# Contingencyy/CPUGPUPathtracing

Hardware: AMD Instinct MI355X
Metric: Mrays/sec @ 1920x1080, 256 spp (dragon glTF stand-in) (higher is better)
Workload: dtype f32

## Files before the change

cpugpupathtracing_amd/_native.py:

```python
from __future__ import annotations

import ctypes as C
import os

from ._paths import LIB_PATH

ABI_VERSION = 2
CGPT_OK, CGPT_ERR_INVALID, CGPT_ERR_HIP, CGPT_ERR_NO_SCENE, CGPT_ERR_UNSUPPORTED, CGPT_ERR_NO_DEVICE = range(6)
OBJECT_MESH, OBJECT_SPHERE, OBJECT_PLANE, OBJECT_TRIANGLE = 0, 1, 2, 3
MODE_COMPARISON, MODE_BRUTE_FORCE, MODE_ADVANCED = 0, 1, 2
DEBUG_NONE, DEBUG_RAY_DEPTH, DEBUG_BVH_DEPTH = 0, 1, 2
KERNEL_AUTO, KERNEL_MEGAKERNEL, KERNEL_WAVEFRONT, KERNEL_PERSISTENT = 0, 1, 2, 3
RENDER_COUNTERS = 1
CTX_FORCE_COLLECTIVE, CTX_GATHER_PEER_COPY = 1, 2
BUILD_NAIVE, BUILD_SAH_INTERVALS, BUILD_SAH_PRIMITIVES = 0, 1, 2
BUILD_SAH_BINNED = 3
DENOISE_DEMODULATE_ALBEDO = 1
TRACE_COUNTERS, TRACE_REVERSED = 1, 2
TEMPORAL_KEEP_VIEW_DEPENDENT = 1
TEMPORAL_FOLLOW_TRANSFORMS = 4
VARIANCE_TEMPORAL = 1
SKIN_MAX_JOINTS = 1024

f3 = C.c_float * 3
# ... 202 lines not shown
    "cgpth_scene_get_smooth_normals": (C.c_int, [_vp, _up, C.c_uint32]),
    "cgpth_scene_set_transform": (C.c_int, [_vp, C.c_uint32, C.POINTER(C.c_float)]),
    "cgpth_scene_get_transforms": (C.c_int, [_vp, C.POINTER(C.c_float), C.c_uint32]),
    "cgpth_scene_set_camera": (C.c_int, [_vp, _fp, _fp, C.c_float, C.c_float]),
    "cgpth_scene_set_settings": (C.c_int, [_vp, C.POINTER(Settings)]),
    "cgpth_scene_rebuild_bvh": (C.c_int, [_vp, C.c_uint32, C.c_int]),
    "cgpth_scene_refit_mesh": (C.c_int, [_vp, C.c_uint32, C.POINTER(Triangle), C.c_uint32]),
    "cgpth_skin_triangles": (C.c_int, [C.POINTER(Triangle), _u16p, _fp, C.c_uint32, _fp, C.c_uint32, C.POINTER(Triangle)]),
    "cgpth_scene_skin_mesh": (C.c_int, [_vp, C.c_uint32, C.POINTER(Triangle), _u16p, _fp, C.c_uint32, _fp, C.c_uint32]),
    "cgpth_scene_update_primitive": (C.c_int, [_vp, C.c_uint32, C.POINTER(Object)]),
    "cgpth_scene_bvh_info": (C.c_int, [_vp, C.c_uint32, C.POINTER(BvhInfo)]),
    "cgpth_scene_bvh_export": (C.c_int, [_vp, C.c_uint32, C.POINTER(BvhNode), _up]),
    "cgpth_scene_flatten": (C.c_int, [_vp, C.POINTER(SceneDesc)]),
    "cgpth_scene_get_camera": (C.c_int, [_vp, C.POINTER(Camera)]),
    "cgpth_scene_get_settings": (C.c_int, [_vp, C.POINTER(Settings)]),
    "cgpth_write_ppm": (C.c_int, [C.c_char_p, _up, C.c_uint32, C.c_uint32]),
    "cgpth_write_pfm": (C.c_int, [C.c_char_p, _fp, C.c_uint32, C.c_uint32, C.c_uint32]),
    "cgpth_write_accumulator": (C.c_int, [C.c_char_p, _fp, C.c_uint32, C.c_uint32, C.c_uint32]),
    "cgpth_read_accumulator": (C.c_int, [C.c_char_p, _fp, _up, C.c_uint32, C.c_uint32]),
    "cgpth_fast_div": (C.c_uint32, [C.c_uint32, C.c_uint32]),
    "cgpth_motion_records": (C.c_uint32, [_fp, C.c_uint32, _fp, C.c_uint32, _fp]),
    "cgpth_shade_item_blocks": (C.c_uint32, [C.c_uint32, C.c_uint32, C.c_uint32]),
    "cgpth_shade_segment_blocks": (C.c_uint32, [C.c_uint32, C.c_uint32, C.c_uint32]),
    "cgpth_scene_layout": (C.c_int, [C.POINTER(SceneDesc), C.POINTER(SceneLayoutView)]),
    "cgpth_scene_layout_instanced": (C.c_int, [C.POINTER(SceneDesc), C.POINTER(SceneLayoutView)]),
    "cgpth_scene_layout_transformed": (C.c_int, [C.POINTER(SceneDesc), C.POINTER(C.c_float), C.c_uint32, C.POINTER(SceneLayoutView)]),
    "cgpth_scene_permute_objects": (C.c_int, [_vp, _up, C.c_uint32]),
    "cgpth_top_level": (C.c_int, [C.POINTER(SceneDesc), C.POINTER(TopLevelView)]),
    "cgpth_top_level_transforms": (C.c_int, [C.POINTER(C.c_float), C.c_uint32, C.POINTER(TopLevelView)]),
    "cgpth_top_level_refit": (C.c_int, [C.c_uint32, C.POINTER(Triangle), C.c_uint32, C.POINTER(TopLevelView)]),
    "cgpth_top_level_primitive": (C.c_int, [C.c_uint32, C.POINTER(Object), C.POINTER(TopLevelView)]),
}

DEBUG_PROTOTYPES = {
    "cgpt_debug_live_device_bytes": (C.c_uint64, []),
}

_lib = None


class NativeLibraryError(RuntimeError):
    pass


def lib() -> C.CDLL:
    global _lib
# ... 19 lines not shown
```

cpugpupathtracing_amd/csrc/device/persistent_kernel.hip:

```cpp
#include <hip/hip_runtime.h>

#include <algorithm>
#include <cstdint>
#include <cstdlib>
#include <new>

#include "cpugpupt_abi.h"
#include "device_scene.h"
#include "fast_div.h"
#include "rt_device.hpp"
#include "shade_device.hpp"
#include "trace_steps.hpp"
#include "accumulate.hpp"
#include "launch_common.h"

namespace cgpt {

using namespace dev;

hipStream_t CtxStream(cgpt_ctx* ctx);
void** CtxPersistentSlot(cgpt_ctx* ctx);
hipEvent_t CtxStartEvent(cgpt_ctx* ctx);
void PersistentFree(void* state);

// ... 359 lines not shown
    LAUNCH_TRY(hipEventRecord(CtxStartEvent(ctx), stream));
    LAUNCH_TRY(hipMemsetAsync(h->work_counters.p, 0, work_words * sizeof(uint32_t), stream));
    const TraceTune tt = { h->tune.refill_idle, h->tune.inner_repeat, h->tune.leaf_repeat, 1u, h->tune.obj_shift, top_records, 0u, h->tune.lds_tris, h->tune.tail_lanes, 0u };

    if (n_streams == 2) {
        LAUNCH_TRY(hipEventRecord(h->begin, stream));
        for (int i = 0; i < 2; ++i) LAUNCH_TRY(hipStreamWaitEvent(h->streams[i], h->begin, 0));
    }
    int launches = 0;
    uint32_t k = 0;
    for (uint32_t done = 0; done < args_in.n_samples; done += batch, ++k) {
        const uint32_t s = n_streams == 2 ? k & 1u : 0u;
        hipStream_t st = n_streams == 2 ? h->streams[s] : stream;
        const uint32_t bn = std::min(batch, args_in.n_samples - done);
        const uint32_t bfirst = args_in.first_sample + done;
        PtDev pt{};
        pt.st_en = h->st_en[s].p;
        pt.brute = brute ? h->brute.p + (size_t)s * (h->brute.n / n_streams) : nullptr;
        pt.stack_overflow = h->overflow.p + (size_t)s * (h->overflow.n / n_streams);
        pt.n_paths = n_pixels * bn;
        pt.g.n_pixels = n_pixels; pt.g.tiles_x = tiles_x; pt.g.div_tiles_x = MakeFastDiv(tiles_x); pt.g.div_n_pixels = MakeFastDiv(n_pixels);
        pt.shade_shift = h->tune.shade_shift;
        pt.g.order = h->tune.path_order; pt.g.n_samples = bn; pt.g.div_samples = MakeFastDiv(bn);
        pt.work = h->work_counters.p + (size_t)k * kWorkCounters * 8u;
        work_sizes(pt.n_paths, grid.x * (kTraceBlock / 64u), h->tune.fine_rounds, h->tune.chunk, pt.coarse, pt.fine_below);
        LAUNCH_TRY(hipEventRecord(NextEvent(h->ev), st));
        hipLaunchKernelGGL(kPtKernels[v.ris][level][v.count][brute][tail], grid, trace_block, lds, st, args_in, pt, bfirst, tt);
        LAUNCH_TRY(hipEventRecord(NextEvent(h->ev), st));
        if (n_streams == 2 && k > 0) LAUNCH_TRY(hipStreamWaitEvent(st, h->acc_done[(k - 1u) & 1u], 0));
        hipLaunchKernelGGL(pt_accumulate, dim3(std::min((n_pixels + 255u) / 256u, h->n_cus * 8u)), block, 0, st, args_in, (const float4*)pt.st_en, pt.g, bfirst, bn);
        if (n_streams == 2) LAUNCH_TRY(hipEventRecord(h->acc_done[s], st));
        LAUNCH_TRY(hipGetLastError());
        launches += 2;
    }
    if (n_streams == 2 && k > 0) LAUNCH_TRY(hipStreamWaitEvent(stream, h->acc_done[(k - 1u) & 1u], 0));
    return launches;
}

}
```

cpugpupathtracing_amd/csrc/device/trace_steps.hpp:

```cpp
#pragma once
#include <hip/hip_runtime.h>

#include "device_scene.h"
#include "fast_div.h"
#include "rt_device.hpp"

namespace cgpt {
namespace dev {

static constexpr uint32_t kStartObject = 0x40000000u;
static constexpr uint32_t kIdle = 0x40000001u;
#ifndef CGPT_LDS_STACK_LEVELS
#define CGPT_LDS_STACK_LEVELS 16
#endif
static constexpr uint32_t kLdsStackLevels = CGPT_LDS_STACK_LEVELS;
#ifndef CGPT_TRACE_BLOCK
#define CGPT_TRACE_BLOCK 256
#endif
static constexpr uint32_t kTraceBlock = CGPT_TRACE_BLOCK;
static constexpr uint32_t kRing = 128;
static constexpr uint32_t kLdsObjects = 31;
static constexpr uint32_t kKindEnd = 0xFFFFFFFFu;
static constexpr uint32_t kTopStride = 20;
static constexpr uint32_t kLdsTopMax = 127;
// ... 60 lines not shown

typedef float nt_f4 __attribute__((ext_vector_type(4)));
__device__ __forceinline__ float4 ld_stream(const float4* p)
{
    const nt_f4 v = __builtin_nontemporal_load(reinterpret_cast<const nt_f4*>(p));
    float4 r; r.x = v.x; r.y = v.y; r.z = v.z; r.w = v.w; return r;
}
__device__ __forceinline__ void st_stream(float4* p, float4 v)
{
    nt_f4 x; x.x = v.x; x.y = v.y; x.z = v.z; x.w = v.w;
    __builtin_nontemporal_store(x, reinterpret_cast<nt_f4*>(p));
}
__device__ __forceinline__ uint32_t ld_stream(const uint32_t* p) { return __builtin_nontemporal_load(p); }
__device__ __forceinline__ void st_stream(uint32_t* p, uint32_t v) { __builtin_nontemporal_store(v, p); }

enum PathOrder : uint32_t { kSampleMajor = 0, kTileMajor = 1, kPixelMajor = 2 };
struct PathGrid {
    uint32_t n_pixels;
    uint32_t tiles_x;
    FastDiv div_tiles_x, div_n_pixels;
    uint32_t n_samples;
    FastDiv div_samples;
    uint32_t order;
};
__device__ __forceinline__ void path_split(const PathGrid& g, uint32_t pid, uint32_t& sample, uint32_t& pixel)
{
    if (g.order == kPixelMajor) {
        pixel = fast_div(pid, g.div_samples);
        sample = pid - pixel * g.n_samples;
    } else if (g.order == kTileMajor) {
        const uint32_t b = pid >> 6, tile = fast_div(b, g.div_samples);
        sample = b - tile * g.n_samples;
        pixel = (tile << 6) | (pid & 63u);
    } else {
        sample = fast_div(pid, g.div_n_pixels);
        pixel = pid - sample * g.n_pixels;
    }
}
__device__ __forceinline__ uint32_t path_id(const PathGrid& g, uint32_t sample, uint32_t pixel)
{
    if (g.order == kPixelMajor) return pixel * g.n_samples + sample;
    return g.order == kTileMajor ? ((((pixel >> 6) * g.n_samples + sample) << 6) | (pixel & 63u)) : sample * g.n_pixels + pixel;
}
__device__ __forceinline__ bool pixel_of_index(const DevRenderArgs& a, const PathGrid& g, uint32_t p, uint32_t& px, uint32_t& py, uint32_t& local_row)
{
    const uint32_t tile = p >> 6, l = p & 63u;
    const uint32_t ty = fast_div(tile, g.div_tiles_x);
    const uint32_t tx = tile - ty * g.tiles_x;
    px = tx * 8u + (l & 7u);
    local_row = ty * 8u + (l >> 3);
    py = GlobalRow(local_row, a.band_first, a.band_h, a.band_stride);
    return px < a.width && local_row < a.n_rows;
}
__device__ __forceinline__ bool primary_ray(const DevRenderArgs& args, const PathGrid& g, uint32_t pid, uint32_t batch_first, Ray& ray, uint32_t& rng, uint32_t& px_out,
                                            uint32_t& pixel_out)
{
    uint32_t s, p;
    path_split(g, pid, s, p);
    pixel_out = p;
    uint32_t px, py, local_row;
    if (!pixel_of_index(args, g, p, px, py, local_row)) return false;
    px_out = px;
    rng = pcg_seed(py * args.width + px, batch_first + s, args.seed);
    ray = camera_ray(args.camera, (float)px * (1.0f / (float)args.width), (float)py * (1.0f / (float)args.height));
    return true;
}
__device__ __forceinline__ bool primary_ray(const DevRenderArgs& args, const PathGrid& g, uint32_t pid, uint32_t batch_first, Ray& ray, uint32_t& rng, uint32_t& px_out)
{
    uint32_t pixel_unused;
    return primary_ray(args, g, pid, batch_first, ray, rng, px_out, pixel_unused);
}
__device__ __forceinline__ bool pixel_ray(const DevRenderArgs& args, const PathGrid& g, uint32_t p, Ray& ray)
{
// ... 330 lines not shown
```

cpugpupathtracing_amd/csrc/device/wavefront_kernels.hip:

```cpp
#include <hip/hip_runtime.h>

#include <algorithm>
#include <cstdint>
#include <cstddef>
#include <cstdlib>
#include <cstring>
#include <new>
#include <type_traits>
#include <vector>

#include "cpugpupt_abi.h"
#include "ctx_internal.h"
#include "device_scene.h"
#include "fast_div.h"
#include "rt_device.hpp"
#include "shade_device.hpp"
#include "shade_items.h"
#include "trace_steps.hpp"
#include "accumulate.hpp"
#include "launch_common.h"

namespace cgpt {

using namespace dev;

hipStream_t CtxStream(cgpt_ctx* ctx);
void** CtxWavefrontSlot(cgpt_ctx* ctx);
hipEvent_t CtxStartEvent(cgpt_ctx* ctx);

extern __shared__ uint32_t lds_dyn[];

static constexpr uint32_t kMaxBands = 128;

struct WfDev {
    float4* A; float4* B; float4* C;
    float4* st_tp; float4* st_en;
    float4* px_hit;
    float4* brute;
    uint8_t* hit_flag;
    uint32_t* list_ext; uint32_t* list_sh;
// ... 557 lines not shown
                off += n; base += total;
            }
            if (seg == 0u) wf.plan[sh ? 1 : 0] = base;
        }
        __syncthreads();
        const uint32_t* src = (sh ? wf.seg_sh : wf.seg_ext) + (size_t)seg * wf.seg_cap;
        uint32_t* const list = sh ? wf.list_sh : wf.list_ext;
        for (uint32_t b = wave_in_block; b < wf.n_bands; b += 4u) {
            const uint32_t n = s_n[b], n4 = n & ~3u;
            uint32_t* dst = list + s_dst[b];
            const uint32_t* run = src + s_src[b];
            for (uint32_t i = lane * 4u; i < n4; i += 256u) *reinterpret_cast<u4a4*>(dst + i) = *reinterpret_cast<const u4a4*>(run + i);
            if (lane < n - n4) dst[n4 + lane] = run[n4 + lane];
        }
    }
}

__global__ void __launch_bounds__(256) wf_accumulate(const DevRenderArgs args, const WfDev wf, uint32_t batch_first, uint32_t batch_n)
{
    accumulate_batch<true>(args, wf.st_en, wf.g, batch_first, batch_n, wf.px_hit);
}

static constexpr uint32_t kMaxPools = 8;

struct WfTuning {
    uint32_t pools = 8;
    uint32_t batch = 0;
    uint32_t max_batch = 512;
    uint32_t pool_paths_mi = 512;
    uint32_t budget_gib = 96;
    uint32_t refill_idle = 16;
    uint32_t leaf_repeat = 4;
    uint32_t inner_repeat = 20;
    uint32_t obj_repeat = 1;
    uint32_t obj_shift = 0;
    uint32_t top_records = kLdsTopMax;
    uint32_t max_trace_blocks = 64;
    uint32_t max_shade_blocks = 5;
    uint32_t shade_chunk = 4;
    uint32_t shade_chunk_banded = 32;
    uint32_t shadow_any_hit = 1;
    uint32_t lds_tris = 1;
    uint32_t first_lean = 1;
    uint32_t trace_events = 1;
    uint32_t path_order = 2;
    uint32_t retire_misses = 1;
    uint32_t bands_min_paths = 32u << 20;
    uint32_t bands = 32;
    uint32_t spec_dedupe = 1;
// ... 49 lines not shown
    f(d.st_tp, paths * sizeof(float4)); f(d.st_en, paths * sizeof(float4)); f(d.hit_flag, paths);
    f(d.px_hit, (size_t)s.n_pixels * sizeof(float4));
    f(d.brute, (size_t)s.brute_levels * paths * 2u * sizeof(float4));
    f(d.list_ext, paths * sizeof(uint32_t)); f(d.list_sh, paths * sizeof(uint32_t));
    f(d.seg_ext, segs); f(d.seg_sh, segs);
    f(d.seg_count, runs); f(d.seg_prefix, runs);
    f(d.plan, (2 + 2 * (size_t)kMaxBands) * sizeof(uint32_t));
    f(d.stack_overflow, (size_t)s.overflow_words * sizeof(uint32_t));
    f(d.spec_tab, s.spec * sizeof(unsigned long long));
}

static size_t PoolBytes(const WfSizes& s)
{
    WfDev d{};
    size_t n = 0;
    ForEachBuffer(d, s, [&](auto*&, size_t bytes) { n += bytes; });
    return n;
}

struct WfHost {
    WfTuning tune;
    WfDev dev[kMaxPools] = {};
    hipStream_t streams[kMaxPools] = {};
    hipEvent_t acc_done[kMaxPools] = {};
    hipEvent_t begin = nullptr;
    WfSizes held;
    uint32_t held_pools = 0;
    uint32_t spec_epoch[kMaxPools] = {};
    uint32_t n_cus = 0;
    uint32_t trace_blocks_per_cu[2][2][2] = {}, shade_blocks_per_cu[2][kLobeLevels][2][2] = {};
    bool last_xform = false;
    uint32_t trace_tree_blocks_per_cu[2][2][2] = {};
    bool last_tree = false;
    size_t occupancy_lds = 0, tree_occupancy_lds = 0;
    EventPairs trace_ev;
    uint32_t trace_rounds = 0;
};

static void WfRelease(WfHost* h)
{
    for (uint32_t p = 0; p < kMaxPools; ++p) {
        ForEachBuffer(h->dev[p], h->held, [](auto*& ptr, size_t) { DevFree(ptr); });
        h->dev[p] = WfDev{};
    }
    h->held = WfSizes{}; h->held_pools = 0;
}

void WavefrontFree(void* state)
{
    if (!state) return;
    WfHost* h = static_cast<WfHost*>(state);
    WfRelease(h);
    for (uint32_t p = 0; p < kMaxPools; ++p) {
        if (h->streams[p]) (void)hipStreamDestroy(h->streams[p]);
        if (h->acc_done[p]) (void)hipEventDestroy(h->acc_done[p]);
    }
    if (h->begin) (void)hipEventDestroy(h->begin);
    FreeEvents(h->trace_ev);
    delete h;
}

uint32_t WavefrontTraceWavesPerSimd(void* state)
{
    if (!state) return 0;
    const WfHost* h = static_cast<const WfHost*>(state);
    return std::min(h->tune.max_trace_blocks, (h->last_tree ? h->trace_tree_blocks_per_cu : h->trace_blocks_per_cu)[h->last_xform][0][0]) * (kTraceBlock / 256u);
}

void WavefrontCollectTiming(void* state, double* trace_ms, uint32_t* trace_launches, double* round0_ms, uint32_t* round0_launches)
{
    *trace_ms = 0.0; *trace_launches = 0; *round0_ms = 0.0; *round0_launches = 0;
    if (!state) return;
    WfHost* h = static_cast<WfHost*>(state);
    ForEachPair(h->trace_ev, [&](uint32_t i, float ms) {
        *trace_ms += ms; *trace_launches += 1;
        if (h->trace_rounds && i % h->trace_rounds == 0u) { *round0_ms += ms; *round0_launches += 1; }
    });
}

static const Knob<WfTuning> kKnobs[] = {
    { "pools", &WfTuning::pools, 1, kMaxPools },           { "batch", &WfTuning::batch, 0, 4096 },
    { "max_batch", &WfTuning::max_batch, 1, 4096 },         { "pool_paths_mi", &WfTuning::pool_paths_mi, 1, 1024 },
    { "budget_gib", &WfTuning::budget_gib, 1, 256 },       { "refill", &WfTuning::refill_idle, 1, 64 },
    { "leaf_repeat", &WfTuning::leaf_repeat, 1, 65 },      { "inner_repeat", &WfTuning::inner_repeat, 1, 65 },
    { "obj_repeat", &WfTuning::obj_repeat, 1, 65 },        { "obj_shift", &WfTuning::obj_shift, 0, 6 },
    { "top_records", &WfTuning::top_records, 0, 4096 },     { "trace_blocks", &WfTuning::max_trace_blocks, 1, 64 },
    { "shade_blocks", &WfTuning::max_shade_blocks, 1, 64 },
    { "shade_chunk", &WfTuning::shade_chunk, 1, 256 },     { "shade_chunk_banded", &WfTuning::shade_chunk_banded, 1, 256 },
    { "shadow_any_hit", &WfTuning::shadow_any_hit, 0, 1 },     { "trace_events", &WfTuning::trace_events, 0, 1 },
    { "path_order", &WfTuning::path_order, 0, 2 },         { "retire_misses", &WfTuning::retire_misses, 0, 1 },
    { "lds_tris", &WfTuning::lds_tris, 0, 1 },             { "first_lean", &WfTuning::first_lean, 0, 1 },                     { "bands", &WfTuning::bands, 1, kMaxBands },             { "bands_min_paths", &WfTuning::bands_min_paths, 0, 0x7FFFFFFF },
    { "spec_dedupe", &WfTuning::spec_dedupe, 0, 1 },       { "spec_keys", &WfTuning::spec_keys, 1, 16 },
    { "spec_epochs", &WfTuning::spec_epochs, 1, 0xFFFF },   { "probe", &WfTuning::probe, 0, 1 },
    { "probe_max_objects", &WfTuning::probe_max_objects, 0, 4096 }, { "probe_lights", &WfTuning::probe_lights, 0, 1 },
};

static WfHost* WfGetHost(cgpt_ctx* ctx)
{
    void** slot = CtxWavefrontSlot(ctx);
    if (*slot) return static_cast<WfHost*>(*slot);
    WfHost* fresh = new (std::nothrow) WfHost;
    if (!fresh) { CtxFail(ctx, CGPT_ERR_INVALID, "out of host memory"); return nullptr; }
    LoadKnobsFromEnv(kKnobs, "CGPT_WF_", fresh->tune);
    hipError_t e = hipEventCreateWithFlags(&fresh->begin, hipEventDisableTiming);
// ... 39 lines not shown
        for (int r = 0; r < 2; ++r)
            for (int g = 0; g < kLobeLevels; ++g)
                for (int c = 0; c < 2; ++c)
                    for (int b = 0; b < 2; ++b) h->shade_blocks_per_cu[r][g][c][b] = std::min(shade[r][g][c][0][b], shade[r][g][c][1][b]);
        h->occupancy_lds = trace_lds;
    }
    if (tree && h->tree_occupancy_lds != trace_lds) {
        LAUNCH_TRY(QueryOccupancy(&kTraceTreeKernels[0][0][0], &h->trace_tree_blocks_per_cu[0][0][0], TableCount(kTraceTreeKernels), kTraceBlock, trace_lds));
        h->tree_occupancy_lds = trace_lds;
    }
    const uint32_t (&trace_blocks)[2][2][2] = tree ? h->trace_tree_blocks_per_cu : h->trace_blocks_per_cu;
    tl.kernels = tree ? kTraceTreeKernels : kTraceKernels;
    tl.grid_first = dim3(n_cus * std::min(h->tune.max_trace_blocks, trace_blocks[xform][count][1]));
    tl.grid_later = dim3(n_cus * std::min(h->tune.max_trace_blocks, trace_blocks[xform][count][0]));
    tl.lds = trace_lds;
    tl.tune = TraceTune{ h->tune.refill_idle, h->tune.inner_repeat, h->tune.leaf_repeat, h->tune.obj_repeat, h->tune.obj_shift, top_records, h->tune.shadow_any_hit, h->tune.lds_tris, 0u, h->tune.first_lean };
    const uint32_t max_trace_threads = n_cus * std::max(*std::max_element(&h->trace_blocks_per_cu[0][0][0], &h->trace_blocks_per_cu[0][0][0] + TableCount(h->trace_blocks_per_cu)),
                                                        *std::max_element(&h->trace_tree_blocks_per_cu[0][0][0], &h->trace_tree_blocks_per_cu[0][0][0] + TableCount(h->trace_tree_blocks_per_cu))) * kTraceBlock;
    const uint32_t deep_levels = sc.stack_depth > kLdsStackLevels ? sc.stack_depth - kLdsStackLevels : 0u;
    tl.overflow_words = std::max(1u, deep_levels * max_trace_threads);
    return 0;
}

static PathGrid MakePathGrid(uint32_t n_pixels, uint32_t tiles_x, uint32_t n_samples, uint32_t order)
{
    PathGrid g{};
    g.n_pixels = n_pixels; g.tiles_x = tiles_x; g.div_tiles_x = MakeFastDiv(tiles_x); g.div_n_pixels = MakeFastDiv(n_pixels);
    g.n_samples = n_samples; g.div_samples = MakeFastDiv(n_samples); g.order = order;
    return g;
}

int LaunchWavefront(cgpt_ctx* ctx, const DevRenderArgs& args_in, ShadeVariant v)
{
    hipStream_t stream = CtxStream(ctx);
    WfHost* h = WfGetHost(ctx);
    if (!h) return -1;
    const bool count = v.count;
    const uint32_t rows = args_in.n_rows;
    const uint32_t tiles_x = (args_in.width + 7u) / 8u, tiles_y = (rows + 7u) / 8u;
    const uint64_t n_pixels64 = (uint64_t)tiles_x * tiles_y * 64u;
    const uint32_t pool_paths = h->tune.pool_paths_mi << 20;
    if (n_pixels64 > pool_paths) { CtxFail(ctx, CGPT_ERR_UNSUPPORTED, "band of %llu pixels exceeds the wavefront pool", (unsigned long long)n_pixels64); return -1; }
    const uint32_t n_pixels = (uint32_t)n_pixels64;
    const uint32_t rounds = (uint32_t)args_in.settings.max_ray_depth + 2u;

    const bool xform = HonoursTransforms((int)v.lobe_level);
    h->last_xform = xform;
    const bool tree = v.tree;
    h->last_tree = tree;
    TraceLaunch tl;
    if (PrepareTraceLaunch(ctx, h, args_in.scene, xform, count, tree, tl) != 0) return -1;
    const uint32_t n_cus = h->n_cus;
    const dim3 block(256);
    const auto& trace_kernels = tl.kernels;
    const size_t trace_lds = tl.lds;
    const dim3 trace_grid_first = tl.grid_first, trace_grid_later = tl.grid_later;
    const bool brute = args_in.settings.render_mode != 2u;
    const uint32_t brute_levels = brute ? (uint32_t)args_in.settings.max_ray_depth + 1u : 0u;
    uint32_t shade_blocks[2][2];
    for (int c = 0; c < 2; ++c)
        for (int b = 0; b < 2; ++b) shade_blocks[c][b] = std::min(h->tune.max_shade_blocks, h->shade_blocks_per_cu[v.ris][v.lobe_level][c][b]);
    const dim3 shade_grid(n_cus * shade_blocks[count][brute]);
    const uint32_t n_segs = n_cus * std::max({ shade_blocks[0][0], shade_blocks[1][0], shade_blocks[0][1], shade_blocks[1][1] }) * 4u;
    const uint32_t min_shade_waves = n_cus * std::min({ shade_blocks[0][0], shade_blocks[1][0], shade_blocks[0][1], shade_blocks[1][1] }) * 4u;

    const uint32_t overflow_words = tl.overflow_words;

    uint32_t shade_chunk = h->tune.shade_chunk;
    const bool chains = h->tune.spec_dedupe && !count && !brute;
    const size_t spec_entries = chains ? (size_t)n_pixels * h->tune.spec_keys : 0u;
    const size_t kBytesPerPath = 160 + 32 * (size_t)brute_levels;
    size_t free_b = 0, total_b = 0;
    LAUNCH_TRY(hipMemGetInfo(&free_b, &total_b));
    const size_t held_bytes = (size_t)h->held_pools * PoolBytes(h->held);
    const size_t budget = std::min<size_t>((size_t)h->tune.budget_gib << 30, (free_b + held_bytes) / 2);
    uint32_t batch = h->tune.batch;
    if (batch == 0) {
        batch = 1;
        while (batch < h->tune.max_batch && (uint64_t)n_pixels * batch * 2u <= (uint64_t)pool_paths) batch *= 2u;
    }
    batch = std::max(1u, std::min({ batch, std::max(1u, args_in.n_samples / 2u), args_in.n_samples, pool_paths / n_pixels }));
    WfSizes need;
    need.n_pixels = n_pixels; need.n_segs = n_segs; need.overflow_words = overflow_words; need.brute_levels = brute_levels; need.spec = spec_entries;
    uint32_t n_pools = 0, n_batches = 0;
    for (int attempt = 0;; ++attempt) {
        for (;;) {
            need.cap = n_pixels * batch;
            n_batches = (args_in.n_samples + batch - 1u) / batch;
            const uint32_t afford = (uint32_t)std::min<size_t>(kMaxPools, budget / ((size_t)need.cap * kBytesPerPath + spec_entries * sizeof(unsigned long long)));
            n_pools = std::max(1u, std::min({ h->tune.pools, n_batches, afford }));
            if (batch == 1u || (afford >= 1u && n_pools >= std::min({ 2u, n_batches, h->tune.pools }))) break;
            batch /= 2u;
        }
        const bool banded = h->tune.bands > 1u && need.cap >= h->tune.bands_min_paths;
        shade_chunk = banded ? h->tune.shade_chunk_banded : h->tune.shade_chunk;
        need.seg_cap = shade_segment_blocks((need.cap + 63u) / 64u, min_shade_waves, shade_chunk) * 64u;
        if (h->held_pools >= n_pools && h->held.Holds(need)) break;
        LAUNCH_TRY(hipDeviceSynchronize());
        WfRelease(h);
        hipError_t err = hipSuccess;
        for (uint32_t p = 0; p < n_pools; ++p) {
            WfDev& d = h->dev[p];
            ForEachBuffer(d, need, [&](auto*& ptr, size_t bytes) { if (err == hipSuccess && bytes) err = DevAlloc((void**)&ptr, bytes); });
            if (err == hipSuccess && d.spec_tab) err = hipMemset(d.spec_tab, 0, need.spec * sizeof(unsigned long long));
            h->spec_epoch[p] = 0;
        }
        if (err == hipSuccess) { h->held = need; h->held_pools = n_pools; break; }
        (void)hipGetLastError();
        WfRelease(h);
        if (batch == 1u || attempt >= 8) { CtxFail(ctx, CGPT_ERR_HIP, "wavefront pools: %s", hipGetErrorString(err)); return -1; }
        batch /= 2u;
    }

    if (ReserveEvents(ctx, h->trace_ev, 2u * n_batches * rounds) != 0) return -1;
    h->trace_rounds = rounds;

    LAUNCH_TRY(hipEventRecord(CtxStartEvent(ctx), stream));
    LAUNCH_TRY(hipEventRecord(h->begin, stream));
    for (uint32_t p = 0; p < n_pools; ++p) LAUNCH_TRY(hipStreamWaitEvent(h->streams[p], h->begin, 0));

    int launches = 0;
    DevRenderArgs args = args_in;
    const TraceTune tt = tl.tune;
    uint32_t k = 0;
    for (uint32_t done = 0; done < args_in.n_samples; done += batch, ++k) {
        const uint32_t p = k % n_pools;
        hipStream_t st = h->streams[p];
        const uint32_t bn = std::min(batch, args_in.n_samples - done);
        const uint32_t bfirst = args_in.first_sample + done;
        WfDev wf = h->dev[p];
        wf.cap = h->held.cap; wf.n_paths = n_pixels * bn;
        wf.rot_trace[0] = CoprimeRotation(trace_grid_later.x * (kTraceBlock / 64u), tiles_x * tiles_y);
        wf.rot_trace[1] = CoprimeRotation(trace_grid_first.x * (kTraceBlock / 64u), tiles_x * tiles_y);
        wf.rot_shade = CoprimeRotation(shade_grid.x * 4u, std::max(1u, tiles_x * tiles_y / shade_chunk));
        wf.shade_chunk = shade_chunk;
        wf.g = MakePathGrid(n_pixels, tiles_x, bn, h->tune.path_order); wf.n_segs = h->held.n_segs; wf.seg_cap = h->held.seg_cap;
        wf.n_bands = h->tune.bands > 1u && wf.n_paths >= h->tune.bands_min_paths ? h->tune.bands : 1u;
        if (wf.n_bands > 1u)
            wf.band_magic = (uint32_t)std::min<uint64_t>(0xFFFFFFFFull, (((uint64_t)wf.n_bands << 32) + wf.n_paths - 1u) / wf.n_paths);
        wf.retire_misses = h->tune.retire_misses && args_in.settings.debug_mode == 0u ? 1u : 0u;
        if (!chains) wf.spec_tab = nullptr;
        wf.spec_keys = h->tune.spec_keys;
        wf.probe = h->tune.probe && !count && !xform && !tree && args_in.settings.debug_mode == 0u && args_in.scene.n_objects <= h->tune.probe_max_objects ? 1u : 0u;
        wf.probe_lights = h->tune.probe_lights;
        if (k < n_pools) LAUNCH_TRY(hipMemsetAsync(wf.seg_count, 0, 2 * (size_t)kMaxBands * wf.n_segs * sizeof(uint32_t), st));
        for (uint32_t r = 0; r < rounds; ++r) {
            const bool first = r == 0u;
            if (h->tune.trace_events) LAUNCH_TRY(hipEventRecord(NextEvent(h->trace_ev), st));
            hipLaunchKernelGGL(trace_kernels[xform][count][first], first ? trace_grid_first : trace_grid_later, dim3(kTraceBlock), trace_lds, st, args, wf, bfirst, tt);
            if (h->tune.trace_events) LAUNCH_TRY(hipEventRecord(NextEvent(h->trace_ev), st));
            ++launches;
            if (r + 1u < rounds) {
                if (wf.spec_tab) {
                    if (++h->spec_epoch[p] > h->tune.spec_epochs) {
                        LAUNCH_TRY(hipMemsetAsync(wf.spec_tab, 0, h->held.spec * sizeof(unsigned long long), st));
                        h->spec_epoch[p] = 1u;
                    }
                    wf.spec_epoch = h->spec_epoch[p];
                }
                hipLaunchKernelGGL(kShadeKernels[v.ris][v.lobe_level][count][first][brute], shade_grid, block, 0, st, args, wf, bfirst);
                hipLaunchKernelGGL(wf_plan, dim3(2u * wf.n_bands), dim3(256), 0, st, wf);
                hipLaunchKernelGGL(wf_gather, dim3(std::min(2u * wf.n_segs, n_cus * 16u)), block, 0, st, wf);
                launches += 3;
            }
        }
        if (k > 0) LAUNCH_TRY(hipStreamWaitEvent(st, h->acc_done[(k - 1u) % n_pools], 0));
        hipLaunchKernelGGL(wf_accumulate, dim3(std::min((n_pixels + 255u) / 256u, n_cus * 8u)), block, 0, st, args, wf, bfirst, bn);
        ++launches;
        LAUNCH_TRY(hipEventRecord(h->acc_done[p], st));
        LAUNCH_TRY(hipGetLastError());
    }
    if (k > 0) LAUNCH_TRY(hipStreamWaitEvent(stream, h->acc_done[(k - 1u) % n_pools], 0));
    return launches;
}

namespace {

constexpr uint32_t kMaxProbeRays = 1u << 22;
constexpr uint32_t kTraceProbeFlags = CGPT_TRACE_COUNTERS | CGPT_TRACE_REVERSED;

float4 F4(float x, float y, float z, float w) { float4 v; v.x = x; v.y = y; v.z = z; v.w = w; return v; }
float BitsToFloat(uint32_t u) { float f; memcpy(&f, &u, sizeof(f)); return f; }
uint32_t FloatToBits(float f) { uint32_t u; memcpy(&u, &f, sizeof(u)); return u; }

struct ProbeSetup { WfHost* h; ShadeVariant v; bool xform; TraceLaunch tl; DevRenderArgs args; };
int ProbeBegin(cgpt_ctx* ctx, uint32_t flags, ProbeSetup& s)
{
    HIP_TRY(ctx, hipSetDevice(ctx->device));
    s.h = WfGetHost(ctx);
    if (!s.h) return CGPT_ERR_HIP;
    s.args = DevRenderArgs{};
    s.args.settings.render_mode = CGPT_MODE_ADVANCED;
    s.v = ChooseVariant(ctx, s.args.settings, (flags & CGPT_TRACE_COUNTERS) ? (uint32_t)CGPT_RENDER_COUNTERS : 0u);
    s.xform = HonoursTransforms((int)s.v.lobe_level);
    if (PrepareTraceLaunch(ctx, s.h, ctx->scene, s.xform, s.v.count, s.v.tree, s.tl) != 0) return CGPT_ERR_HIP;
// ... 162 lines not shown
```

cpugpupathtracing_amd/csrc/host/host_capi.cpp:

```cpp
#include <cstring>
#include <exception>
#include <new>
#include <string>
#include <vector>

#include "cpugpupt_host.h"
#include "fast_div.h"
#include "gltf_loader.h"
#include "image_io.h"
#include "mesh_gen.h"
#include "scene.h"
#include "shade_items.h"
#include "skinning.h"
#include "transform_math.h"

using namespace cgpt;

struct cgpth_mesh { Mesh mesh; };
struct cgpth_scene {
    Scene scene;
    Scene::FlatStorage flat;
};

namespace {
thread_local std::string g_error;
int Fail(const std::string& msg) { g_error = msg; return CGPT_ERR_INVALID; }
Vec3 V(const float p[3]) { return { p[0], p[1], p[2] }; }

Material FromAbi(const cgpt_material& m)
{
    Material out;
    out.albedo = V(m.albedo); out.specular = m.specular; out.refractivity = m.refractivity;
    out.absorption = V(m.absorption); out.ior = m.ior; out.emissive = V(m.emissive);
    out.intensity = m.intensity; out.is_light = m.is_light != 0;
    return out;
// ... 539 lines not shown
}
int cgpth_write_accumulator(const char* path, const float* acc, uint32_t n, uint32_t width, uint32_t height)
{
    return Guarded<int>((int)CGPT_ERR_INVALID, [&]() -> int {
        std::string err;
        if (!path || !acc) return Fail("null argument");
        return WriteAccumulator(path, acc, n, width, height, err) ? CGPT_OK : Fail(err);
    });
}
int cgpth_read_accumulator(const char* path, float* acc, uint32_t* n, uint32_t width, uint32_t height)
{
    return Guarded<int>((int)CGPT_ERR_INVALID, [&]() -> int {
        std::string err;
        if (!path || !acc || !n) return Fail("null argument");
        return ReadAccumulator(path, acc, n, width, height, err) ? CGPT_OK : Fail(err);
    });
}

uint32_t cgpth_fast_div(uint32_t n, uint32_t d) { return d == 0u ? 0u : fast_div(n, MakeFastDiv(d)); }

uint32_t cgpth_shade_item_blocks(uint32_t n_blocks, uint32_t n_waves, uint32_t chunk) { return n_waves == 0u || chunk == 0u ? 0u : shade_item_blocks(n_blocks, n_waves, chunk); }
uint32_t cgpth_shade_segment_blocks(uint32_t cap_blocks, uint32_t min_waves, uint32_t chunk) { return min_waves == 0u || chunk == 0u ? 0u : shade_segment_blocks(cap_blocks, min_waves, chunk); }

uint32_t cgpth_motion_records(const float* prev, uint32_t n_prev, const float* cur, uint32_t n_objects, float* records_out)
{
    if (!prev || !cur || !records_out) return 0u;
    static_assert(sizeof(MotionRecord) == 24 * sizeof(float), "24 words per object");
    return (uint32_t)CompareTransforms(prev, n_prev, cur, n_objects, reinterpret_cast<MotionRecord*>(records_out));
}

}
```

include/cpugpupt_host.h:

```cpp
#ifndef CPUGPUPT_HOST_H
#define CPUGPUPT_HOST_H

#include "cpugpupt_abi.h"

#ifdef __cplusplus
extern "C" {
#endif

enum cgpth_build_option { CGPTH_BUILD_NAIVE = 0, CGPTH_BUILD_SAH_INTERVALS = 1, CGPTH_BUILD_SAH_PRIMITIVES = 2,
                          CGPTH_BUILD_SAH_BINNED = 3  };

typedef struct cgpth_mesh cgpth_mesh;
typedef struct cgpth_scene cgpth_scene;

typedef struct cgpth_bvh_info {
    uint32_t num_triangles, nodes_used, num_leaves, max_leaf_size, max_depth;
    float total_area;
} cgpth_bvh_info;

const char* cgpth_last_error(void);

cgpth_mesh* cgpth_mesh_load_gltf(const char* path);
cgpth_mesh* cgpth_mesh_from_arrays(const cgpt_vertex* vertices, uint32_t n_vertices, const uint32_t* indices, uint32_t n_indices);
cgpth_mesh* cgpth_mesh_dragon_standin(uint32_t level);
// ... 33 lines not shown
int cgpth_scene_refit_mesh(cgpth_scene* scene, uint32_t obj_index, const cgpt_triangle* triangles, uint32_t n_tris);
int cgpth_skin_triangles(const cgpt_triangle* bind_triangles, const uint16_t* joints, const float* weights, uint32_t n_tris,
                         const float* joint_matrices, uint32_t n_joints, cgpt_triangle* out_triangles);
int cgpth_scene_skin_mesh(cgpth_scene* scene, uint32_t obj_index, const cgpt_triangle* bind_triangles, const uint16_t* joints, const float* weights,
                          uint32_t n_tris, const float* joint_matrices, uint32_t n_joints);
int cgpth_scene_update_primitive(cgpth_scene* scene, uint32_t obj_index, const cgpt_object* obj);
int cgpth_scene_permute_objects(cgpth_scene* scene, const uint32_t* order, uint32_t n_objects);
int cgpth_scene_bvh_info(const cgpth_scene* scene, uint32_t obj_index, cgpth_bvh_info* out);
int cgpth_scene_bvh_export(const cgpth_scene* scene, uint32_t obj_index, cgpt_bvh_node* nodes, uint32_t* tri_indices);
int cgpth_scene_flatten(cgpth_scene* scene, cgpt_scene_desc* out);
int cgpth_scene_get_camera(const cgpth_scene* scene, cgpt_camera* out);
int cgpth_scene_get_settings(const cgpth_scene* scene, cgpt_settings* out);

int cgpth_write_ppm(const char* path, const uint32_t* pixels, uint32_t width, uint32_t height);
int cgpth_write_pfm(const char* path, const float* accumulator_rgba, uint32_t num_accumulated, uint32_t width, uint32_t height);
int cgpth_write_accumulator(const char* path, const float* accumulator_rgba, uint32_t num_accumulated, uint32_t width, uint32_t height);
int cgpth_read_accumulator(const char* path, float* accumulator_rgba, uint32_t* num_accumulated, uint32_t width, uint32_t height);

uint32_t cgpth_fast_div(uint32_t n, uint32_t d);

uint32_t cgpth_shade_item_blocks(uint32_t n_blocks, uint32_t n_waves, uint32_t chunk);
uint32_t cgpth_shade_segment_blocks(uint32_t cap_blocks, uint32_t min_waves, uint32_t chunk);

uint32_t cgpth_motion_records(const float* prev, uint32_t n_prev, const float* cur, uint32_t n_objects, float* records_out);

typedef struct cgpth_scene_layout_view {
    const float* node_pairs; size_t n_node_pairs;
    const float* tri_leaf; size_t n_tri_leaf;
    const float* tri_orig; size_t n_tri_orig;
    const float* tri_normal; size_t n_tri_normal;
    const float* materials; size_t n_materials;
    const float* obj_trace; size_t n_obj_trace;
    const void* objects; size_t n_objects; size_t object_size;
    const uint32_t* lights; size_t n_lights;
    const uint32_t* refit_levels; size_t n_refit_levels;
    const uint32_t* record_perm; size_t n_record_perm;
    uint32_t stack_depth, n_top_records, n_pair_records, n_small_tris;
    const uint32_t* leaf_base; const uint32_t* pair_base; const uint32_t* level_begin;
    const uint32_t* level_offsets; const uint32_t* level_offsets_start;
    const float* tri_normal12; size_t n_tri_normal12;
    const float* obj_xform; size_t n_obj_xform;
} cgpth_scene_layout_view;
int cgpth_scene_layout(const cgpt_scene_desc* scene, cgpth_scene_layout_view* out);
int cgpth_scene_layout_instanced(const cgpt_scene_desc* scene, cgpth_scene_layout_view* out);
int cgpth_scene_layout_transformed(const cgpt_scene_desc* scene, const float* object_to_world, uint32_t n_objects, cgpth_scene_layout_view* out);

// ... 14 lines not shown
```

Measured before the change: 23250.

## Split wavefront render into interleaved tile-row strips as independent work units

Adds strip partitioning of tile rows, so each sample batch is issued per strip with its own path grid mapping, rotations, shade chunk and accumulate event. When the frame has many paths, it automatically uses two strips and lets a batch cover all samples. The aim is to shrink each unit's working set and change scheduling across pools. The cost is extra per-unit launches and memsets, plus cross-strip event dependencies.

After: 23190. No clear change (-0.2%).

```diff
diff --git a/cpugpupathtracing_amd/_native.py b/cpugpupathtracing_amd/_native.py
--- a/cpugpupathtracing_amd/_native.py
+++ b/cpugpupathtracing_amd/_native.py
@@ -248,6 +248,10 @@
     "cgpth_motion_records": (C.c_uint32, [_fp, C.c_uint32, _fp, C.c_uint32, _fp]),
     "cgpth_shade_item_blocks": (C.c_uint32, [C.c_uint32, C.c_uint32, C.c_uint32]),
     "cgpth_shade_segment_blocks": (C.c_uint32, [C.c_uint32, C.c_uint32, C.c_uint32]),
+    "cgpth_strip_tile_rows": (C.c_uint32, [C.c_uint32, C.c_uint32, C.c_uint32]),
+    "cgpth_strip_tile_row": (C.c_uint32, [C.c_uint32, C.c_uint32, C.c_uint32]),
+    "cgpth_strip_count": (C.c_uint32, [C.c_uint32, C.c_uint32]),
+    "cgpth_strip_auto_count": (C.c_uint32, [C.c_uint64]),
     "cgpth_scene_layout": (C.c_int, [C.POINTER(SceneDesc), C.POINTER(SceneLayoutView)]),
     "cgpth_scene_layout_instanced": (C.c_int, [C.POINTER(SceneDesc), C.POINTER(SceneLayoutView)]),
     "cgpth_scene_layout_transformed": (C.c_int, [C.POINTER(SceneDesc), C.POINTER(C.c_float), C.c_uint32, C.POINTER(SceneLayoutView)]),
diff --git a/cpugpupathtracing_amd/csrc/device/persistent_kernel.hip b/cpugpupathtracing_amd/csrc/device/persistent_kernel.hip
--- a/cpugpupathtracing_amd/csrc/device/persistent_kernel.hip
+++ b/cpugpupathtracing_amd/csrc/device/persistent_kernel.hip
@@ -405,6 +405,7 @@
         pt.g.n_pixels = n_pixels; pt.g.tiles_x = tiles_x; pt.g.div_tiles_x = MakeFastDiv(tiles_x); pt.g.div_n_pixels = MakeFastDiv(n_pixels);
         pt.shade_shift = h->tune.shade_shift;
         pt.g.order = h->tune.path_order; pt.g.n_samples = bn; pt.g.div_samples = MakeFastDiv(bn);
+        pt.g.tile_row_mul = 1u; pt.g.tile_row_add = 0u;
         pt.work = h->work_counters.p + (size_t)k * kWorkCounters * 8u;
         work_sizes(pt.n_paths, grid.x * (kTraceBlock / 64u), h->tune.fine_rounds, h->tune.chunk, pt.coarse, pt.fine_below);
         LAUNCH_TRY(hipEventRecord(NextEvent(h->ev), st));
diff --git a/cpugpupathtracing_amd/csrc/device/strip_units.h b/cpugpupathtracing_amd/csrc/device/strip_units.h
--- /dev/null
+++ b/cpugpupathtracing_amd/csrc/device/strip_units.h
@@ -0,0 +1,29 @@
+#pragma once
+#include <cstdint>
+
+#include "fast_div.h"
+
+namespace cgpt {
+
+CGPT_HD inline uint32_t strip_tile_rows(uint32_t T, uint32_t K, uint32_t j)
+{
+    return j < T ? (T - j - 1u) / K + 1u : 0u;
+}
+
+CGPT_HD inline uint32_t strip_tile_row(uint32_t K, uint32_t j, uint32_t i)
+{
+    return j + K * i;
+}
+
+CGPT_HD inline uint32_t strip_count(uint32_t T, uint32_t K)
+{
+    return K < T ? (K ? K : 1u) : (T ? T : 1u);
+}
+
+static constexpr uint64_t kStripAutoMinPaths = 384ull << 20;
+CGPT_HD inline uint32_t strip_auto_count(uint64_t n_paths)
+{
+    return n_paths >= kStripAutoMinPaths ? 2u : 1u;
+}
+
+}
diff --git a/cpugpupathtracing_amd/csrc/device/trace_steps.hpp b/cpugpupathtracing_amd/csrc/device/trace_steps.hpp
--- a/cpugpupathtracing_amd/csrc/device/trace_steps.hpp
+++ b/cpugpupathtracing_amd/csrc/device/trace_steps.hpp
@@ -106,6 +106,7 @@
     uint32_t n_samples;
     FastDiv div_samples;
     uint32_t order;
+    uint32_t tile_row_mul, tile_row_add;
 };
 __device__ __forceinline__ void path_split(const PathGrid& g, uint32_t pid, uint32_t& sample, uint32_t& pixel)
 {
@@ -132,7 +133,7 @@
     const uint32_t ty = fast_div(tile, g.div_tiles_x);
     const uint32_t tx = tile - ty * g.tiles_x;
     px = tx * 8u + (l & 7u);
-    local_row = ty * 8u + (l >> 3);
+    local_row = (ty * g.tile_row_mul + g.tile_row_add) * 8u + (l >> 3);
     py = GlobalRow(local_row, a.band_first, a.band_h, a.band_stride);
     return px < a.width && local_row < a.n_rows;
 }
diff --git a/cpugpupathtracing_amd/csrc/device/wavefront_kernels.hip b/cpugpupathtracing_amd/csrc/device/wavefront_kernels.hip
--- a/cpugpupathtracing_amd/csrc/device/wavefront_kernels.hip
+++ b/cpugpupathtracing_amd/csrc/device/wavefront_kernels.hip
@@ -16,6 +16,7 @@
 #include "rt_device.hpp"
 #include "shade_device.hpp"
 #include "shade_items.h"
+#include "strip_units.h"
 #include "trace_steps.hpp"
 #include "accumulate.hpp"
 #include "launch_common.h"
@@ -619,9 +620,11 @@
 }
 
 static constexpr uint32_t kMaxPools = 8;
+static constexpr uint32_t kMaxStrips = 64;
 
 struct WfTuning {
     uint32_t pools = 8;
+    uint32_t strips = 0;
     uint32_t batch = 0;
     uint32_t max_batch = 512;
     uint32_t pool_paths_mi = 512;
@@ -717,7 +720,7 @@
     WfTuning tune;
     WfDev dev[kMaxPools] = {};
     hipStream_t streams[kMaxPools] = {};
-    hipEvent_t acc_done[kMaxPools] = {};
+    hipEvent_t acc_done[kMaxStrips] = {};
     hipEvent_t begin = nullptr;
     WfSizes held;
     uint32_t held_pools = 0;
@@ -746,10 +749,10 @@
     if (!state) return;
     WfHost* h = static_cast<WfHost*>(state);
     WfRelease(h);
-    for (uint32_t p = 0; p < kMaxPools; ++p) {
+    for (uint32_t p = 0; p < kMaxPools; ++p)
         if (h->streams[p]) (void)hipStreamDestroy(h->streams[p]);
-        if (h->acc_done[p]) (void)hipEventDestroy(h->acc_done[p]);
-    }
+    for (uint32_t j = 0; j < kMaxStrips; ++j)
+        if (h->acc_done[j]) (void)hipEventDestroy(h->acc_done[j]);
     if (h->begin) (void)hipEventDestroy(h->begin);
     FreeEvents(h->trace_ev);
     delete h;
@@ -775,6 +778,7 @@
 
 static const Knob<WfTuning> kKnobs[] = {
     { "pools", &WfTuning::pools, 1, kMaxPools },           { "batch", &WfTuning::batch, 0, 4096 },
+    { "strips", &WfTuning::strips, 0, kMaxStrips },
     { "max_batch", &WfTuning::max_batch, 1, 4096 },         { "pool_paths_mi", &WfTuning::pool_paths_mi, 1, 1024 },
     { "budget_gib", &WfTuning::budget_gib, 1, 256 },       { "refill", &WfTuning::refill_idle, 1, 64 },
     { "leaf_repeat", &WfTuning::leaf_repeat, 1, 65 },      { "inner_repeat", &WfTuning::inner_repeat, 1, 65 },
@@ -860,11 +864,12 @@
     return 0;
 }
 
-static PathGrid MakePathGrid(uint32_t n_pixels, uint32_t tiles_x, uint32_t n_samples, uint32_t order)
+static PathGrid MakePathGrid(uint32_t n_pixels, uint32_t tiles_x, uint32_t n_samples, uint32_t order, uint32_t strips = 1u, uint32_t strip = 0u)
 {
     PathGrid g{};
     g.n_pixels = n_pixels; g.tiles_x = tiles_x; g.div_tiles_x = MakeFastDiv(tiles_x); g.div_n_pixels = MakeFastDiv(n_pixels);
     g.n_samples = n_samples; g.div_samples = MakeFastDiv(n_samples); g.order = order;
+    g.tile_row_mul = strips; g.tile_row_add = strip_tile_row(strips, strip, 0u);
     return g;
 }
 
@@ -876,10 +881,15 @@
     const bool count = v.count;
     const uint32_t rows = args_in.n_rows;
     const uint32_t tiles_x = (args_in.width + 7u) / 8u, tiles_y = (rows + 7u) / 8u;
-    const uint64_t n_pixels64 = (uint64_t)tiles_x * tiles_y * 64u;
+    const uint32_t auto_strips = args_in.n_samples <= h->tune.max_batch ? strip_auto_count((uint64_t)tiles_x * tiles_y * 64u * args_in.n_samples) : 1u;
+    const uint32_t n_strips = strip_count(tiles_y, h->tune.strips ? h->tune.strips : auto_strips);
+    const uint64_t n_pixels64 = (uint64_t)tiles_x * strip_tile_rows(tiles_y, n_strips, 0u) * 64u;
     const uint32_t pool_paths = h->tune.pool_paths_mi << 20;
     if (n_pixels64 > pool_paths) { CtxFail(ctx, CGPT_ERR_UNSUPPORTED, "band of %llu pixels exceeds the wavefront pool", (unsigned long long)n_pixels64); return -1; }
     const uint32_t n_pixels = (uint32_t)n_pixels64;
+    const uint32_t max_pools = h->tune.pools;
+    for (uint32_t j = kMaxPools; j < n_strips; ++j)
+        if (!h->acc_done[j]) LAUNCH_TRY(hipEventCreateWithFlags(&h->acc_done[j], hipEventDisableTiming));
     const uint32_t rounds = (uint32_t)args_in.settings.max_ray_depth + 2u;
 
     const bool xform = HonoursTransforms((int)v.lobe_level);
@@ -904,7 +914,6 @@
 
     const uint32_t overflow_words = tl.overflow_words;
 
-    uint32_t shade_chunk = h->tune.shade_chunk;
     const bool chains = h->tune.spec_dedupe && !count && !brute;
     const size_t spec_entries = chains ? (size_t)n_pixels * h->tune.spec_keys : 0u;
     const size_t kBytesPerPath = 160 + 32 * (size_t)brute_levels;
@@ -917,22 +926,28 @@
         batch = 1;
         while (batch < h->tune.max_batch && (uint64_t)n_pixels * batch * 2u <= (uint64_t)pool_paths) batch *= 2u;
     }
-    batch = std::max(1u, std::min({ batch, std::max(1u, args_in.n_samples / 2u), args_in.n_samples, pool_paths / n_pixels }));
+    batch = std::max(1u, std::min({ batch, n_strips > 1u ? args_in.n_samples : std::max(1u, args_in.n_samples / 2u), args_in.n_samples, pool_paths / n_pixels }));
     WfSizes need;
     need.n_pixels = n_pixels; need.n_segs = n_segs; need.overflow_words = overflow_words; need.brute_levels = brute_levels; need.spec = spec_entries;
-    uint32_t n_pools = 0, n_batches = 0;
+    auto unit_banded = [&](uint32_t n_paths) { return h->tune.bands > 1u && n_paths >= h->tune.bands_min_paths; };
+    auto unit_chunk = [&](uint32_t n_paths) { return unit_banded(n_paths) ? h->tune.shade_chunk_banded : h->tune.shade_chunk; };
+    uint32_t n_pools = 0, n_units = 0;
     for (int attempt = 0;; ++attempt) {
         for (;;) {
             need.cap = n_pixels * batch;
-            n_batches = (args_in.n_samples + batch - 1u) / batch;
+            n_units = n_strips * ((args_in.n_samples + batch - 1u) / batch);
             const uint32_t afford = (uint32_t)std::min<size_t>(kMaxPools, budget / ((size_t)need.cap * kBytesPerPath + spec_entries * sizeof(unsigned long long)));
-            n_pools = std::max(1u, std::min({ h->tune.pools, n_batches, afford }));
-            if (batch == 1u || (afford >= 1u && n_pools >= std::min({ 2u, n_batches, h->tune.pools }))) break;
+            n_pools = std::max(1u, std::min({ max_pools, n_units, afford }));
+            if (batch == 1u || (afford >= 1u && n_pools >= std::min({ 2u, n_units, max_pools }))) break;
             batch /= 2u;
         }
-        const bool banded = h->tune.bands > 1u && need.cap >= h->tune.bands_min_paths;
-        shade_chunk = banded ? h->tune.shade_chunk_banded : h->tune.shade_chunk;
-        need.seg_cap = shade_segment_blocks((need.cap + 63u) / 64u, min_shade_waves, shade_chunk) * 64u;
+        need.seg_cap = 0;
+        const uint32_t last_bn = args_in.n_samples % batch;
+        for (uint32_t j = 0; j < n_strips; j += std::max(1u, n_strips - 1u))
+            for (uint32_t bn : { batch, last_bn ? last_bn : batch }) {
+                const uint32_t paths = strip_tile_rows(tiles_y, n_strips, j) * tiles_x * 64u * bn;
+                need.seg_cap = std::max(need.seg_cap, shade_segment_blocks((paths + 63u) / 64u, min_shade_waves, unit_chunk(paths)) * 64u);
+            }
         if (h->held_pools >= n_pools && h->held.Holds(need)) break;
         LAUNCH_TRY(hipDeviceSynchronize());
         WfRelease(h);
@@ -950,7 +965,7 @@
         batch /= 2u;
     }
 
-    if (ReserveEvents(ctx, h->trace_ev, 2u * n_batches * rounds) != 0) return -1;
+    if (ReserveEvents(ctx, h->trace_ev, 2u * n_units * rounds) != 0) return -1;
     h->trace_rounds = rounds;
 
     LAUNCH_TRY(hipEventRecord(CtxStartEvent(ctx), stream));
@@ -960,20 +975,24 @@
     int launches = 0;
     DevRenderArgs args = args_in;
     const TraceTune tt = tl.tune;
+    uint32_t pool_bands[kMaxPools] = {};
     uint32_t k = 0;
-    for (uint32_t done = 0; done < args_in.n_samples; done += batch, ++k) {
+    for (uint32_t done = 0; done < args_in.n_samples; done += batch)
+    for (uint32_t strip = 0; strip < n_strips; ++strip, ++k) {
         const uint32_t p = k % n_pools;
         hipStream_t st = h->streams[p];
         const uint32_t bn = std::min(batch, args_in.n_samples - done);
         const uint32_t bfirst = args_in.first_sample + done;
+        const uint32_t unit_tiles = tiles_x * strip_tile_rows(tiles_y, n_strips, strip), unit_pixels = unit_tiles * 64u;
         WfDev wf = h->dev[p];
-        wf.cap = h->held.cap; wf.n_paths = n_pixels * bn;
-        wf.rot_trace[0] = CoprimeRotation(trace_grid_later.x * (kTraceBlock / 64u), tiles_x * tiles_y);
-        wf.rot_trace[1] = CoprimeRotation(trace_grid_first.x * (kTraceBlock / 64u), tiles_x * tiles_y);
-        wf.rot_shade = CoprimeRotation(shade_grid.x * 4u, std::max(1u, tiles_x * tiles_y / shade_chunk));
+        wf.cap = h->held.cap; wf.n_paths = unit_pixels * bn;
+        const uint32_t shade_chunk = unit_chunk(wf.n_paths);
+        wf.rot_trace[0] = CoprimeRotation(trace_grid_later.x * (kTraceBlock / 64u), unit_tiles);
+        wf.rot_trace[1] = CoprimeRotation(trace_grid_first.x * (kTraceBlock / 64u), unit_tiles);
+        wf.rot_shade = CoprimeRotation(shade_grid.x * 4u, std::max(1u, unit_tiles / shade_chunk));
         wf.shade_chunk = shade_chunk;
-        wf.g = MakePathGrid(n_pixels, tiles_x, bn, h->tune.path_order); wf.n_segs = h->held.n_segs; wf.seg_cap = h->held.seg_cap;
-        wf.n_bands = h->tune.bands > 1u && wf.n_paths >= h->tune.bands_min_paths ? h->tune.bands : 1u;
+        wf.g = MakePathGrid(unit_pixels, tiles_x, bn, h->tune.path_order, n_strips, strip); wf.n_segs = h->held.n_segs; wf.seg_cap = h->held.seg_cap;
+        wf.n_bands = unit_banded(wf.n_paths) ? h->tune.bands : 1u;
         if (wf.n_bands > 1u)
             wf.band_magic = (uint32_t)std::min<uint64_t>(0xFFFFFFFFull, (((uint64_t)wf.n_bands << 32) + wf.n_paths - 1u) / wf.n_paths);
         wf.retire_misses = h->tune.retire_misses && args_in.settings.debug_mode == 0u ? 1u : 0u;
@@ -981,7 +1000,8 @@
         wf.spec_keys = h->tune.spec_keys;
         wf.probe = h->tune.probe && !count && !xform && !tree && args_in.settings.debug_mode == 0u && args_in.scene.n_objects <= h->tune.probe_max_objects ? 1u : 0u;
         wf.probe_lights = h->tune.probe_lights;
-        if (k < n_pools) LAUNCH_TRY(hipMemsetAsync(wf.seg_count, 0, 2 * (size_t)kMaxBands * wf.n_segs * sizeof(uint32_t), st));
+        if (pool_bands[p] != wf.n_bands) LAUNCH_TRY(hipMemsetAsync(wf.seg_count, 0, 2 * (size_t)kMaxBands * wf.n_segs * sizeof(uint32_t), st));
+        pool_bands[p] = wf.n_bands;
         for (uint32_t r = 0; r < rounds; ++r) {
             const bool first = r == 0u;
             if (h->tune.trace_events) LAUNCH_TRY(hipEventRecord(NextEvent(h->trace_ev), st));
@@ -1002,13 +1022,13 @@
                 launches += 3;
             }
         }
-        if (k > 0) LAUNCH_TRY(hipStreamWaitEvent(st, h->acc_done[(k - 1u) % n_pools], 0));
-        hipLaunchKernelGGL(wf_accumulate, dim3(std::min((n_pixels + 255u) / 256u, n_cus * 8u)), block, 0, st, args, wf, bfirst, bn);
+        if (done > 0) LAUNCH_TRY(hipStreamWaitEvent(st, h->acc_done[strip], 0));
+        hipLaunchKernelGGL(wf_accumulate, dim3(std::min((unit_pixels + 255u) / 256u, n_cus * 8u)), block, 0, st, args, wf, bfirst, bn);
         ++launches;
-        LAUNCH_TRY(hipEventRecord(h->acc_done[p], st));
+        LAUNCH_TRY(hipEventRecord(h->acc_done[strip], st));
         LAUNCH_TRY(hipGetLastError());
     }
-    if (k > 0) LAUNCH_TRY(hipStreamWaitEvent(stream, h->acc_done[(k - 1u) % n_pools], 0));
+    for (uint32_t strip = 0; k > 0 && strip < n_strips; ++strip) LAUNCH_TRY(hipStreamWaitEvent(stream, h->acc_done[strip], 0));
     return launches;
 }
 
diff --git a/cpugpupathtracing_amd/csrc/host/host_capi.cpp b/cpugpupathtracing_amd/csrc/host/host_capi.cpp
--- a/cpugpupathtracing_amd/csrc/host/host_capi.cpp
+++ b/cpugpupathtracing_amd/csrc/host/host_capi.cpp
@@ -11,6 +11,7 @@
 #include "mesh_gen.h"
 #include "scene.h"
 #include "shade_items.h"
+#include "strip_units.h"
 #include "skinning.h"
 #include "transform_math.h"
 
@@ -596,6 +597,11 @@
 uint32_t cgpth_shade_item_blocks(uint32_t n_blocks, uint32_t n_waves, uint32_t chunk) { return n_waves == 0u || chunk == 0u ? 0u : shade_item_blocks(n_blocks, n_waves, chunk); }
 uint32_t cgpth_shade_segment_blocks(uint32_t cap_blocks, uint32_t min_waves, uint32_t chunk) { return min_waves == 0u || chunk == 0u ? 0u : shade_segment_blocks(cap_blocks, min_waves, chunk); }
 
+uint32_t cgpth_strip_tile_rows(uint32_t tile_rows, uint32_t strips, uint32_t strip) { return strips == 0u ? 0u : strip_tile_rows(tile_rows, strips, strip); }
+uint32_t cgpth_strip_tile_row(uint32_t strips, uint32_t strip, uint32_t row) { return strip_tile_row(strips, strip, row); }
+uint32_t cgpth_strip_count(uint32_t tile_rows, uint32_t strips) { return strip_count(tile_rows, strips); }
+uint32_t cgpth_strip_auto_count(uint64_t n_paths) { return strip_auto_count(n_paths); }
+
 uint32_t cgpth_motion_records(const float* prev, uint32_t n_prev, const float* cur, uint32_t n_objects, float* records_out)
 {
     if (!prev || !cur || !records_out) return 0u;
diff --git a/include/cpugpupt_host.h b/include/cpugpupt_host.h
--- a/include/cpugpupt_host.h
+++ b/include/cpugpupt_host.h
@@ -79,6 +79,11 @@
 uint32_t cgpth_shade_item_blocks(uint32_t n_blocks, uint32_t n_waves, uint32_t chunk);
 uint32_t cgpth_shade_segment_blocks(uint32_t cap_blocks, uint32_t min_waves, uint32_t chunk);
 
+uint32_t cgpth_strip_tile_rows(uint32_t tile_rows, uint32_t strips, uint32_t strip);
+uint32_t cgpth_strip_tile_row(uint32_t strips, uint32_t strip, uint32_t row);
+uint32_t cgpth_strip_count(uint32_t tile_rows, uint32_t strips);
+uint32_t cgpth_strip_auto_count(uint64_t n_paths);
+
 uint32_t cgpth_motion_records(const float* prev, uint32_t n_prev, const float* cur, uint32_t n_objects, float* records_out);
 
 typedef struct cgpth_scene_layout_view {
```
